# jasonleebrown/machisplin

Hardware: AMD Instinct MI355X
Metric: grid Mcells/s (ensemble+TPS predict) + TPS-solve GFLOP/s (higher is better)
Workload: dtype f64; 1 GPU; cfg3: 5000 stations, 3 covariates, 10000x10000 grid, 6-model ensemble + TPS residual correction; stations=5000, covariates=3 x float32 planes resident in HBM, rf_trees=500, tps_mode=global (one fit on all stations, GCV lambda, V73:748-753), parallelism=rowband1 + bcast(coef) + 1 all-gather

## Files before the change

machisplin_amd/csrc/ensemble.hip:

```cpp
#include <algorithm>
#include <atomic>
#include <chrono>
#include <cmath>
#include <cstdio>
#include <cstdlib>
#include <cstring>
#include <functional>
#include <mutex>
#include <type_traits>
#include <vector>
#include "common.h"
#include "devmath.h"

#include "ensemble_int.h"

namespace mhs {

__global__ __launch_bounds__(256) void lm_kernel(const double *__restrict__ coef, int p, StackDev s,
                                                 PredGeom g, double weight, int accumulate,
                                                 double *__restrict__ out) {
    const int64_t i = (int64_t)blockIdx.x * 256 + threadIdx.x;
    if (i >= (int64_t)g.nr * g.nc) return;
    const int row = (int)(i / g.nc), col = (int)(i - (int64_t)row * g.nc);
    double acc = coef[0];
// ... 64 lines not shown
    double w_lm, w_nn, w_ea;
};
template <int P>
__global__ __launch_bounds__(256) void small_members_kernel(SmallArgs a, StackDev s, PredGeom g, int accumulate,
                                                            double *__restrict__ out) {
    const int64_t i = (int64_t)blockIdx.x * 256 + threadIdx.x;
    if (i >= (int64_t)g.nr * g.nc) return;
    const int row = (int)(i / g.nc), col = (int)(i - (int64_t)row * g.nc);
    double x[P];
    bool na = false;
#pragma unroll
    for (int j = 0; j < P; ++j) { x[j] = predictor(s, g, j, row, col); na |= isnan(x[j]); }
    const int64_t o = (int64_t)row * g.ld_out + col;
    double v = accumulate ? out[o] : 0.0;
    bool first = !accumulate;
    auto add = [&](double pred, double w) { const double t = pred * w; v = first ? t : v + t; first = false; };
    if (a.lm_coef) {
        double acc = a.lm_coef[0];
#pragma unroll
        for (int j = 0; j < P; ++j) acc = acc + a.lm_coef[j + 1] * x[j];
        add(acc, a.w_lm);
    }
    if (a.nn_w) {
        double acc = a.nn_w[(P + 1) * a.nn_H];
        for (int h = 0; h < a.nn_H; ++h) {
            const double *wh = a.nn_w + h * (P + 1);
            double z = wh[0];
#pragma unroll
            for (int j = 0; j < P; ++j) z = z + wh[1 + j] * x[j];
            acc = acc + a.nn_w[(P + 1) * a.nn_H + 1 + h] * nnet_sigmoid(z);
        }
        acc = acc * a.nn_scale + a.nn_shift;
        add(na ? NAN : acc, a.w_nn);
    }
    if (a.ea_coef) {
        double acc = 0.0;
        for (int k = 0; k < a.ea_nterms; ++k) {
            double term = 1.0;
            for (int f = a.ea_tstart[k]; f < a.ea_tstart[k + 1]; ++f) {
                const double xv = predictor(s, g, a.ea_fvar[f], row, col);
                const int d = a.ea_fdir[f];
                const double fac = d == 2 ? xv : (d == 1 ? fmax(0.0, xv - a.ea_cut[f]) : fmax(0.0, a.ea_cut[f] - xv));
                term = term * fac;
            }
            acc = acc + a.ea_coef[k] * term;
        }
        add(na ? NAN : acc, a.w_ea);
    }
    out[o] = v;
}

constexpr int EXP_TAB_BITS = 12;
constexpr int EXP_TAB_N = 1 << EXP_TAB_BITS;
constexpr double EXP_SCALE = 4096.0 / 0.6931471805599453094;
constexpr double EXP_RANGE = 700.0;
__device__ __forceinline__ double table_exp_neg_acc(double u, const double *tab, double acc) {
    const double MAGIC = 0x1.8p52 + 1023.0 * EXP_TAB_N, NK = -EXP_RANGE * EXP_SCALE;
    const double t = fma(u, NK, MAGIC);
    const double kd = t - MAGIC;
    unsigned k8 = (unsigned)__double2loint(t) << 8;
    asm("" : "+v"(k8));
    const double r = fma(u, NK, -kd);
    const double mj = *(const double *)((const char *)tab + __builtin_amdgcn_ubfe(k8, 5, EXP_TAB_BITS + 3));
    const double sj = __hiloint2double((int)((k8 & 0xfff00000u) | (unsigned)__double2hiint(mj)), __double2loint(mj));
    const double C1 = 1.0 / EXP_SCALE, C2 = 0.5 / (EXP_SCALE * EXP_SCALE);
    double q = fma(r, C2, C1);
    q = fma(q, r, 1.0);
    return fma(sj, q, acc);
}

template <int P, int R>
__global__ __launch_bounds__(256) void svr_kernel(const double *__restrict__ svp, int nsv, int stride,
                                                  int npos, const double *__restrict__ xcs,
                                                  const double *__restrict__ gtab, double sigma, double b,
                                                  double amax,
                                                  double y_center, double y_scale, StackDev s, PredGeom g,
                                                  double weight, int accumulate, double *__restrict__ out) {
    __shared__ double etab[EXP_TAB_N];
    for (int i = threadIdx.x; i < EXP_TAB_N; i += 256) {
        const double e = gtab[i];
        etab[i] = __hiloint2double(__double2hiint(e) & 0x000fffff, __double2loint(e));
    }
    __syncthreads();
    const int64_t total = (int64_t)g.nr * g.nc;
    const int64_t half = (total + R - 1) / R;
    const int64_t i0 = (int64_t)blockIdx.x * 256 + threadIdx.x;
    if (i0 >= half) return;
    double x[R][P], q[R], acc[R];
    bool na[R];
    int row[R], col[R];
#pragma unroll
    for (int c = 0; c < R; ++c) {
        int64_t i = i0 + c * half;
        if (i >= total) i = total - 1;
        row[c] = (int)(i / g.nc); col[c] = (int)(i - (int64_t)row[c] * g.nc);
        na[c] = false; q[c] = 0.0; acc[c] = 0.0;
#pragma unroll
        for (int j = 0; j < P; ++j) {
            const double xv = predictor(s, g, j, row[c], col[c]);
            na[c] |= isnan(xv);
            x[c][j] = (xv - xcs[j]) / xcs[P + j];
            q[c] = fma(x[c][j], x[c][j], q[c]);
        }
        q[c] = (sigma / EXP_RANGE) * q[c];
    }
    double accn[R];
#pragma unroll
    for (int c = 0; c < R; ++c) accn[c] = 0.0;
    auto sum_range = [&](int v0, int v1, double (&a)[R]) {
        for (int v = v0; v < v1; ++v) {
            const double *sp = svp + (int64_t)v * stride;
#pragma unroll
            for (int c = 0; c < R; ++c) {
                double arg = q[c] + fma(sp[P - 1], x[c][P - 1], sp[P]);
#pragma unroll
                for (int j = 0; j < P - 1; ++j) arg = fma(sp[j], x[c][j], arg);
                arg = fmin(fmax(arg, 0.0), 1.0);
                a[c] = table_exp_neg_acc(arg, etab, a[c]);
            }
        }
    };
    sum_range(0, npos, acc);
    sum_range(npos, nsv, accn);
#pragma unroll
    for (int c = 0; c < R; ++c) {
        const int64_t i = i0 + c * half;
        if (i < total) {
            const double pred = ((acc[c] - accn[c]) * amax - b) * y_scale + y_center;
            emit(out, (int64_t)row[c] * g.ld_out + col[c], na[c] ? NAN : pred, weight, accumulate);
        }
    }
}

template <int P, int R>
__global__ __launch_bounds__(256) void svr_rt_kernel(const double *__restrict__ svp, int nsv, int stride,
                                                     int npos, const double *__restrict__ xcs,
                                                     const double *__restrict__ gtab, double sigma, double b,
                                                     double amax, double y_center, double y_scale, StackDev s, PredGeom g,
                                                     int tiles_per_row, double weight, int accumulate, double *__restrict__ out) {
    constexpr int CH = 128;
    __shared__ double etab[EXP_TAB_N];
    __shared__ double aw[4][CH];
    for (int i = threadIdx.x; i < EXP_TAB_N; i += 256) {
        const double e = gtab[i];
        etab[i] = __hiloint2double(__double2hiint(e) & 0x000fffff, __double2loint(e));
    }
    __syncthreads();
    const int wave = threadIdx.x >> 6, lane = threadIdx.x & 63;
    const int64_t ntiles = (int64_t)g.nr * tiles_per_row;
    const int64_t tile = (int64_t)blockIdx.x * 4 + wave;
    if (tile >= ntiles) return;
    const int row = (int)(tile / tiles_per_row), tcol = (int)(tile - (int64_t)row * tiles_per_row) * (64 * R);
    double x[R][P], q[R], acc[R], accn[R];
    bool na[R], ok[R];
    int col[R];
#pragma unroll
    for (int c = 0; c < R; ++c) {
        const int cc = tcol + c * 64 + lane;
        ok[c] = cc < g.nc;
        col[c] = min(cc, g.nc - 1);
        na[c] = false; q[c] = 0.0; acc[c] = 0.0; accn[c] = 0.0;
#pragma unroll
        for (int j = 0; j < P; ++j) {
            const double xv = predictor(s, g, j, row, col[c]);
            na[c] |= isnan(xv);
            x[c][j] = (xv - xcs[j]) / xcs[P + j];
            q[c] = fma(x[c][j], x[c][j], q[c]);
        }
        q[c] = (sigma / EXP_RANGE) * q[c];
    }
    const double xlat = x[0][P - 1];
    double qhi = -1.0, qlo = 2e300;
#pragma unroll
    for (int c = 0; c < R; ++c) { qhi = fmax(qhi, q[c]); qlo = fmin(qlo, q[c]); }
#pragma unroll
    for (int o = 32; o > 0; o >>= 1) { qhi = fmax(qhi, __shfl_xor(qhi, o)); qlo = fmin(qlo, __shfl_xor(qlo, o)); }
    const bool fold = __builtin_amdgcn_readfirstlane((int)(qhi - qlo <= 0.5)) != 0;
    const double S = fold ? qhi : 0.0;
    auto sum_range = [&](int v0, int v1, double (&a)[R], auto folded) {
        constexpr bool FOLD = decltype(folded)::value;
        auto pair = [&](const double *sp, const double ap) {
#pragma unroll
            for (int c = 0; c < R; ++c) {
                double arg = FOLD ? ap : q[c] + ap;
#pragma unroll
                for (int j = 0; j < P - 1; ++j) arg = fma(sp[j], x[c][j], arg);
                arg = fmin(fmax(arg, 0.0), 1.0);
                a[c] = table_exp_neg_acc(arg, etab, a[c]);
            }
        };
        for (int vb = v0; vb < v1; vb += CH) {
            const int n = min(CH, v1 - vb);
            __builtin_amdgcn_wave_barrier();
            for (int e = lane; e < n; e += 64) {
                const double *sp = svp + (int64_t)(vb + e) * stride;
                aw[wave][e] = fma(sp[P - 1], xlat, sp[P]) + S;
            }
            __builtin_amdgcn_wave_barrier();
            const double *sp = svp + (int64_t)vb * stride;
            const double *ar = aw[wave];
            int e = 0;
            for (; e + 4 <= n; e += 4) {
#pragma unroll
                for (int k = 0; k < 4; ++k) pair(sp + (int64_t)k * stride, ar[e + k]);
                sp += (int64_t)4 * stride;
            }
            for (; e < n; ++e) { pair(sp, ar[e]); sp += stride; }
        }
    };
    if (fold) {
        sum_range(0, npos, acc, std::true_type());
        sum_range(npos, nsv, accn, std::true_type());
    } else {
        sum_range(0, npos, acc, std::false_type());
        sum_range(npos, nsv, accn, std::false_type());
    }
#pragma unroll
    for (int c = 0; c < R; ++c)
        if (ok[c]) {
            const double back = fold ? exp(EXP_RANGE * (S - q[c])) : 1.0;
            const double pred = ((acc[c] - accn[c]) * back * amax - b) * y_scale + y_center;
            emit(out, (int64_t)row * g.ld_out + col[c], na[c] ? NAN : pred, weight, accumulate);
        }
}

template <bool GBM, bool LDS_NODES, int R, bool NA_ONLY, bool SPLIT = false>
__global__ __launch_bounds__(256) void tree_kernel(const Node *__restrict__ gnodes,
                                                   const int *__restrict__ tree_off,
                                                   const TreeChunk *__restrict__ chunks, int n_chunks,
                                                   int n_trees, double init_f, int p, StackDev s,
                                                   PredGeom g, double weight, int accumulate,
                                                   double *__restrict__ out, const unsigned *__restrict__ na_gate = nullptr) {
    extern __shared__ __attribute__((aligned(16))) char smem[];
    if (NA_ONLY && na_gate && na_gate[1] == 0u) return;
    double *xs = (double *)smem;
    Node *lnodes = (Node *)(smem + (size_t)p * R * 256 * sizeof(double));
    const int64_t total = (int64_t)g.nr * g.nc;
    const int64_t half = (total + R - 1) / R;
    const int64_t i0 = (int64_t)blockIdx.x * 256 + threadIdx.x;
    int row[R], col[R];
    bool na[R];
    double acc[R];
#pragma unroll
    for (int c = 0; c < R; ++c) {
        int64_t i = i0 + c * half;
        if (i >= total) i = total - 1;
        if (i < 0) i = 0;
        row[c] = (int)(i / g.nc); col[c] = (int)(i - (int64_t)row[c] * g.nc);
        na[c] = false; acc[c] = 0.0;
        for (int j = 0; j < p; ++j) {
            const double xv = predictor(s, g, j, row[c], col[c]);
            na[c] |= isnan(xv);
            xs[(j * R + c) * 256 + threadIdx.x] = xv;
        }
    }
    if (NA_ONLY) {
        bool any = false;
#pragma unroll
        for (int c = 0; c < R; ++c) any |= na[c] && i0 < half && (i0 + c * half) < total;
        if (!__syncthreads_or(any)) return;
    }
    int ch_begin = 0, ch_end = n_chunks;
    if (SPLIT) {
        const int per = (n_chunks + (int)gridDim.y - 1) / (int)gridDim.y;
        ch_begin = min((int)blockIdx.y * per, n_chunks);
        ch_end = min(ch_begin + per, n_chunks);
    }
    for (int ch = ch_begin; ch < ch_end; ++ch) {
        const TreeChunk tc = chunks[ch];
        if (LDS_NODES) {
            __syncthreads();
            const int4 *src = (const int4 *)(gnodes + tc.node_begin);
            int4 *dst = (int4 *)lnodes;
            for (int e = threadIdx.x; e < tc.node_count; e += 256) dst[e] = src[e];
            __syncthreads();
        }
        for (int t = tc.first_tree; t < tc.first_tree + tc.n_trees; ++t) {
            const int tbase = LDS_NODES ? tree_off[t] - tc.node_begin : tree_off[t];
#pragma unroll
            for (int c = 0; c < R; ++c) {
                if (NA_ONLY && !na[c]) continue;
                Node nd;
                if constexpr (LDS_NODES) nd = lnodes[tbase]; else nd = gnodes[tbase];
                while (nd.var >= 0) {
                    const double xv = xs[(nd.var * R + c) * 256 + threadIdx.x];
                    unsigned nxt;
                    if (GBM) nxt = isnan(xv) ? nd.missing : (xv < nd.val ? nd.left : nd.right);
                    else nxt = (xv <= nd.val) ? nd.left : nd.right;
                    if constexpr (LDS_NODES) nd = lnodes[tbase + nxt]; else nd = gnodes[tbase + nxt];
                }
                acc[c] = acc[c] + nd.val;
            }
        }
    }
    if (SPLIT) {
#pragma unroll
        for (int c = 0; c < R; ++c) {
            const int64_t i = i0 + c * half;
            if (i0 < half && i < total) out[(int64_t)blockIdx.y * total + i] = (!GBM && na[c]) ? NAN : acc[c];
        }
        return;
    }
#pragma unroll
    for (int c = 0; c < R; ++c) {
        const int64_t i = i0 + c * half;
        if (i0 < half && i < total && (!NA_ONLY || na[c])) {
            double pred;
            if (GBM) pred = init_f + acc[c];
            else pred = na[c] ? NAN : acc[c] / (double)n_trees;
            emit(out, (int64_t)row[c] * g.ld_out + col[c], pred, weight, accumulate);
        }
    }
}


__global__ __launch_bounds__(256) void na_collect_kernel(StackDev s, PredGeom g, unsigned cap, unsigned *__restrict__ list) {
    const int64_t total = (int64_t)g.nr * g.nc;
    const int64_t i = (int64_t)blockIdx.x * 256 + threadIdx.x;
    if (i >= total) return;
    const int row = (int)(i / g.nc), col = (int)(i - (int64_t)row * g.nc);
    bool na = false;
    for (int j = 0; j < s.C; ++j) na |= isnan(predictor(s, g, j, row, col));
    if (na) {
        const unsigned slot = atomicAdd(&list[0], 1u);
        if (slot < cap) list[2 + slot] = (unsigned)i;
        else list[1] = 1u;
    }
}
template <bool LDS_NODES>
__global__ __launch_bounds__(256) void gbm_na_list_kernel(const Node *__restrict__ gnodes, const int *__restrict__ tree_off,
                                                          const TreeChunk *__restrict__ chunks, int n_chunks, double init_f, int p,
                                                          StackDev s, PredGeom g, double weight, int accumulate,
                                                          double *__restrict__ out, const unsigned *__restrict__ list, unsigned cap) {
    extern __shared__ __attribute__((aligned(16))) char smem[];
    if (list[1]) return;
    double *xs = (double *)smem;
    Node *lnodes = (Node *)(smem + (size_t)p * 256 * sizeof(double));
    const unsigned count = min(list[0], cap);
    for (unsigned base = blockIdx.x * 256u; base < count; base += gridDim.x * 256u) {
        const bool live = base + threadIdx.x < count;
        const int64_t i = list[2 + (live ? base + threadIdx.x : base)];
        const int row = (int)(i / g.nc), col = (int)(i - (int64_t)row * g.nc);
        for (int j = 0; j < p; ++j) xs[j * 256 + threadIdx.x] = predictor(s, g, j, row, col);
        double acc = 0.0;
        for (int ch = 0; ch < n_chunks; ++ch) {
            const TreeChunk tc = chunks[ch];
            if (LDS_NODES) {
                __syncthreads();
                const int4 *src = (const int4 *)(gnodes + tc.node_begin);
                int4 *dst = (int4 *)lnodes;
                for (int e = threadIdx.x; e < tc.node_count; e += 256) dst[e] = src[e];
                __syncthreads();
            }
            for (int t = tc.first_tree; t < tc.first_tree + tc.n_trees; ++t) {
                const int tbase = LDS_NODES ? tree_off[t] - tc.node_begin : tree_off[t];
                Node nd;
                if constexpr (LDS_NODES) nd = lnodes[tbase]; else nd = gnodes[tbase];
                while (nd.var >= 0) {
                    const double xv = xs[nd.var * 256 + threadIdx.x];
                    const unsigned nxt = isnan(xv) ? nd.missing : (xv < nd.val ? nd.left : nd.right);
                    if constexpr (LDS_NODES) nd = lnodes[tbase + nxt]; else nd = gnodes[tbase + nxt];
                }
                acc = acc + nd.val;
            }
        }
        if (live) emit(out, (int64_t)row * g.ld_out + col, init_f + acc, weight, accumulate);
        __syncthreads();
    }
}


template <bool HI>
__device__ __forceinline__ void pred_bits(float2v &b01, float2v &b23, const float2v k01, const float2v k23,
                                          const unsigned long long cpair) {
    if (!HI)
        asm("v_pk_add_f32 %0, %2, %4 op_sel_hi:[1,0] clamp\n\t"
// ... 452 lines not shown
        const unsigned abase = (unsigned)buf * (unsigned)((CH << S) * sizeof(double)) - 0x58000000u;
        for (unsigned long long m2 = __builtin_amdgcn_ballot_w64(multi); m2; m2 &= m2 - 1ull) {
            const int t = (int)__builtin_ctzll(m2);
            const int n = __builtin_amdgcn_readlane((int)nstr, t);
            const float a0 = __uint_as_float(0x4B000000u + ((unsigned)t << S) + (unsigned)__builtin_amdgcn_readlane((int)known, t));
            float2v s01 = {a0, a0}, s23 = {a0, a0};
#pragma unroll
            for (int l = 0; l < S; ++l) {
                if (l < n) {
                    const unsigned long long cc = (unsigned)__builtin_amdgcn_readlane((int)cl[l], t);
                    const unsigned vw = (unsigned)__builtin_amdgcn_readlane((int)vl[l], t);
                    const int vo = (int)(vw & 0xFFu);
                    const unsigned long long wb = (127u + (vw >> 8)) << 23;
                    float2v b01, b23;
                    asm volatile("s_set_gpr_idx_on %[vo], 0x1\n\t"
                                 "v_pk_add_f32 %[b01], v[64:65], %[cc] op_sel_hi:[1,0] clamp\n\t"
                                 "v_pk_add_f32 %[b23], v[66:67], %[cc] op_sel_hi:[1,0] clamp\n\t"
                                 "s_set_gpr_idx_off\n\t"
                                 "v_pk_fma_f32 %[s01], %[b01], %[wb], %[s01] op_sel_hi:[1,0,1]\n\t"
                                 "v_pk_fma_f32 %[s23], %[b23], %[wb], %[s23] op_sel_hi:[1,0,1]"
                                 : [s01] "+v"(s01), [s23] "+v"(s23), [b01] "=&v"(b01), [b23] "=&v"(b23)
                                 : "{v[64:95]}"(keys), [vo] "s"(vo), [cc] "s"(cc), [wb] "s"(wb));
                }
            }
            acc[0] = acc[0] + gbc_lds_f64(__float_as_uint(s01.x) * 8u + abase);
            acc[1] = acc[1] + gbc_lds_f64(__float_as_uint(s01.y) * 8u + abase);
            acc[2] = acc[2] + gbc_lds_f64(__float_as_uint(s23.x) * 8u + abase);
            acc[3] = acc[3] + gbc_lds_f64(__float_as_uint(s23.y) * 8u + abase);
        }
        if (more) {
            double *ld = slut + (buf ^ 1) * (CH << S);
            ld[tid] = pre0; ld[tid + 1024] = pre1;
            if (tid < CH * S) scls[(buf ^ 1) * CLS_STRIDE + tid] = prec;
        }
        __syncthreads();
    }
    if (PROBE) {
        int *tot = (int *)srange;
        __syncthreads();
        if (tid == 0) tot[0] = 0;
        __syncthreads();
#pragma unroll
        for (int o = 32; o > 0; o >>= 1) pcost += __shfl_xor(pcost, o);
        if (lane == 0) atomicAdd(tot, pcost);
        __syncthreads();
        if (tid == 0) { probe[2 * blockIdx.x] = tot[0]; probe[2 * blockIdx.x + 1] = GBC_WAVES * n_trees_padded; }
        return;
    }
#pragma unroll
    for (int o = 32; o > 0; o >>= 1) usum = usum + __shfl_xor(usum, o);
#pragma unroll
    for (int c = 0; c < R; ++c)
        if (ok[c] && !na[c]) emit(out, (int64_t)row[c] * g.ld_out + col[c], init_f + (acc[c] + usum), weight, accumulate);
}
static size_t gbc_lds_bytes() {
    return 2 * ((size_t)LUT_CHUNK << 5) * sizeof(double) + 2 * 384 * sizeof(unsigned) + GBC_WAVES * 8 * sizeof(int2);
}

__global__ __launch_bounds__(256) void gbm_staged_points_kernel(const Node *__restrict__ nodes, const int *__restrict__ tree_off,
                                                                int n_trees, double init_f, const double *__restrict__ X,
                                                                int64_t n, int step, double *__restrict__ out) {
    const int64_t i = (int64_t)blockIdx.x * 256 + threadIdx.x;
    if (i >= n) return;
    double acc = 0.0;
    for (int t = 0; t < n_trees; ++t) {
        const int tb = tree_off[t];
        Node nd = nodes[tb];
        while (nd.var >= 0) {
            const double xv = X[(int64_t)nd.var * n + i];
            const unsigned nxt = isnan(xv) ? nd.missing : (xv < nd.val ? nd.left : nd.right);
            nd = nodes[tb + nxt];
        }
        acc = acc + nd.val;
        if ((t + 1) % step == 0) out[(int64_t)((t + 1) / step - 1) * n + i] = init_f + acc;
    }
}

struct ResidualArgs { double w[8]; };
__global__ __launch_bounds__(256) void residual_points_kernel(const double *__restrict__ pred, const double *__restrict__ resp,
                                                              int64_t n, int n_models, ResidualArgs a, double wt_total,
                                                              double *__restrict__ out) {
    const int64_t i = (int64_t)blockIdx.x * 256 + threadIdx.x;
    if (i >= n) return;
    const double y = resp[i];
    double res = (y - pred[i]) * a.w[0];
    for (int k = 1; k < n_models; ++k) res = res + (y - pred[(int64_t)k * n + i]) * a.w[k];
    out[i] = res / wt_total;
}

__global__ __launch_bounds__(256) void scale_add_kernel(const double *__restrict__ a, double divisor,
                                                        const double *__restrict__ b,
                                                        double *__restrict__ out, int64_t n) {
    const int64_t i = (int64_t)blockIdx.x * 256 + threadIdx.x;
    if (i >= n) return;
    double v = a[i] / divisor;
    if (b) v = v + b[i];
    out[i] = v;
}

__global__ __launch_bounds__(256) void scale_window_kernel(double *__restrict__ out, int nr, int nc,
                                                           int64_t ld, double divisor) {
    const int64_t i = (int64_t)blockIdx.x * 256 + threadIdx.x;
    if (i >= (int64_t)nr * nc) return;
    const int row = (int)(i / nc), col = (int)(i - (int64_t)row * nc);
    out[(int64_t)row * ld + col] = out[(int64_t)row * ld + col] / divisor;
}


int finish_trees(mhs_model *m, const std::vector<Node> &nodes, const std::vector<int> &off) {
    const int nt = m->n_trees;
    const size_t xs_bytes = (size_t)m->p * TREE_R * 256 * sizeof(double);
    int biggest = 0;
    for (int t = 0; t < nt; ++t) biggest = std::max(biggest, off[t + 1] - off[t]);
    int cap = (m->kind == K_GBM) ? std::max(GBM_CHUNK_NODES, biggest) : biggest;
    m->lds_ok = xs_bytes + (size_t)cap * sizeof(Node) <= LDS_LIMIT;
    std::vector<TreeChunk> chunks;
    if (m->lds_ok) {
        int t = 0;
        while (t < nt) {
            TreeChunk c{t, 0, off[t], 0};
            while (t < nt && off[t + 1] - c.node_begin <= cap) { ++t; }
            c.n_trees = t - c.first_tree;
            c.node_count = off[t] - c.node_begin;
            chunks.push_back(c);
        }
        m->max_chunk_nodes = cap;
    } else {
        chunks.push_back(TreeChunk{0, nt, 0, off[nt]});
        m->max_chunk_nodes = 0;
    }
    m->n_chunks = (int)chunks.size();
    m->n_nodes = (int64_t)nodes.size();
    if (int rc = to_device(nodes.data(), nodes.size(), &m->nodes)) return rc;
    if (int rc = to_device(off.data(), off.size(), &m->tree_off)) return rc;
    return to_device(chunks.data(), chunks.size(), &m->chunks);
}

int check_common(int p, mhs_model **out) {
    if (int rc = require_ready()) return rc;
    MHS_REQUIRE(out != nullptr, "out is NULL");
    MHS_REQUIRE(p >= 2 && p <= 64, "p (covariates + LONG + LAT) out of range");
    return MHS_OK;
}

template <int P>
static void launch_nnet(const mhs_model *m, const StackDev &s, const PredGeom &g, double w, int acc,
                        double *out, hipStream_t st, unsigned blocks) {
    hipLaunchKernelGGL((nnet_kernel<P>), dim3(blocks), dim3(256), 0, st, m->dpar, m->n0, m->s0, m->s1, s, g, w, acc, out);
}
template <int P>
static void launch_svr(const mhs_model *m, const StackDev &s, const PredGeom &g, double w, int acc,
                       double *out, hipStream_t st, int64_t total) {
    constexpr int R = 3;
    const int tpr = (g.nc + 64 * R - 1) / (64 * R);
    if (!s.all_from_planes && P == s.C + 2 && P >= 3 && !getenv("MHS_SVR_NO_ROWTILE") && (double)g.nc >= 0.93 * (double)tpr * (64 * R)) {
        const int64_t ntiles = (int64_t)g.nr * tpr;
        hipLaunchKernelGGL((svr_rt_kernel<P, R>), dim3((unsigned)((ntiles + 3) / 4)), dim3(256), 0, st,
                           m->dpar, m->n0, m->n1, m->n2, m->dpar + (size_t)m->n0 * m->n1, ctx().exp_tab, m->s1, m->s0, m->s4,
                           m->s2, m->s3, s, g, tpr, w, acc, out);
        return;
    }
    const int64_t half = (total + R - 1) / R;
    hipLaunchKernelGGL((svr_kernel<P, R>), dim3((unsigned)((half + 255) / 256)), dim3(256), 0, st,
                       m->dpar, m->n0, m->n1, m->n2, m->dpar + (size_t)m->n0 * m->n1, ctx().exp_tab, m->s1, m->s0, m->s4,
                       m->s2, m->s3,
                       s, g, w, acc, out);
}

#define MHS_DISPATCH_P(P_, CALL)                                                     \
    switch (P_) {                                                                    \
        case 2: CALL(2); break; case 3: CALL(3); break; case 4: CALL(4); break;      \
        case 5: CALL(5); break; case 6: CALL(6); break; case 7: CALL(7); break;      \
        case 8: CALL(8); break; case 9: CALL(9); break; case 10: CALL(10); break;    \
        case 11: CALL(11); break; case 12: CALL(12); break;                          \
        default: set_error("predict: p = %d exceeds the %d predictors this build supports for nnet/ksvm", P_, PMAX); \
                 return MHS_ERR_INVALID;                                             \
    }

template <bool GBM>
__global__ __launch_bounds__(256) void tree_finalize_kernel(const double *__restrict__ part, int shares, int64_t total,
                                                            double init_f, int n_trees, PredGeom g, double weight,
                                                            int accumulate, double *__restrict__ out) {
    const int64_t i = (int64_t)blockIdx.x * 256 + threadIdx.x;
    if (i >= total) return;
    double acc = 0.0;
    for (int y = 0; y < shares; ++y) acc = acc + part[(int64_t)y * total + i];
    const int row = (int)(i / g.nc), col = (int)(i - (int64_t)row * g.nc);
    emit(out, (int64_t)row * g.ld_out + col, GBM ? init_f + acc : acc / (double)n_trees, weight, accumulate);
}

constexpr int64_t TREE_SPLIT_MAX_CELLS = 16384;
constexpr int TREE_SPLIT_SHARES = 64;

template <bool GBM, bool NA_ONLY>
static int launch_trees(const mhs_model *m, const StackDev &s, const PredGeom &g, double w, int acc,
                        double *out, hipStream_t st, int64_t total) {
    const int64_t half = (total + TREE_R - 1) / TREE_R;
    const unsigned blocks = (unsigned)((half + 255) / 256);
    const size_t xs_bytes = (size_t)m->p * TREE_R * 256 * sizeof(double);
    if (!NA_ONLY && m->lds_ok && total <= TREE_SPLIT_MAX_CELLS && m->n_chunks >= 4) {
        const int shares = std::min(m->n_chunks, TREE_SPLIT_SHARES);
        mhs_model *mm = const_cast<mhs_model *>(m);
        if (!mm->split_scratch) MHS_HIP(hipMalloc((void **)&mm->split_scratch, sizeof(double) * TREE_SPLIT_MAX_CELLS * TREE_SPLIT_SHARES));
        const size_t bytes = xs_bytes + (size_t)m->max_chunk_nodes * sizeof(Node);
        auto kern = tree_kernel<GBM, true, TREE_R, false, true>;
        MHS_HIP(hipFuncSetAttribute((const void *)kern, hipFuncAttributeMaxDynamicSharedMemorySize, (int)bytes));
        hipLaunchKernelGGL(kern, dim3(blocks, (unsigned)shares), dim3(256), bytes, st, m->nodes, m->tree_off, m->chunks,
                           m->n_chunks, m->n_trees, m->init_f, m->p, s, g, w, acc, mm->split_scratch, (const unsigned *)nullptr);
        hipLaunchKernelGGL(tree_finalize_kernel<GBM>, dim3((unsigned)((total + 255) / 256)), dim3(256), 0, st,
                           mm->split_scratch, shares, total, m->init_f, m->n_trees, g, w, acc, out);
        return MHS_OK;
    }
    if (m->lds_ok) {
        const size_t bytes = xs_bytes + (size_t)m->max_chunk_nodes * sizeof(Node);
        auto kern = tree_kernel<GBM, true, TREE_R, NA_ONLY>;
        MHS_HIP(hipFuncSetAttribute((const void *)kern, hipFuncAttributeMaxDynamicSharedMemorySize, (int)bytes));
        hipLaunchKernelGGL(kern, dim3(blocks), dim3(256), bytes, st, m->nodes, m->tree_off, m->chunks,
                           m->n_chunks, m->n_trees, m->init_f, m->p, s, g, w, acc, out, (const unsigned *)nullptr);
    } else {
        auto kern = tree_kernel<GBM, false, TREE_R, NA_ONLY>;
        MHS_HIP(hipFuncSetAttribute((const void *)kern, hipFuncAttributeMaxDynamicSharedMemorySize, (int)xs_bytes));
        hipLaunchKernelGGL(kern, dim3(blocks), dim3(256), xs_bytes, st, m->nodes, m->tree_off, m->chunks,
                           m->n_chunks, m->n_trees, m->init_f, m->p, s, g, w, acc, out, (const unsigned *)nullptr);
    }
    return MHS_OK;
}

template <typename KT>
static int build_lut_meta_t(mhs_model *m, const mhs_grid &grid, int C) {
    const int S = m->lut_S;
    std::vector<KT> tkey((size_t)m->n_trees * S, (KT)0);
    std::vector<std::vector<KT>> sorted((size_t)m->p);
    for (int t = 0; t < m->n_trees; ++t) {
        for (int q = 0; q < S; ++q) {
            const int v = m->lut_var[(size_t)t * S + q];
            if (v < 0) continue;
            const KT tk = split_tkey<KT, false>(v, C, m->lut_thr[(size_t)t * S + q], grid);
            tkey[(size_t)t * S + q] = tk;
            sorted[(size_t)v].push_back(tk);
        }
    }
    std::vector<int> off;
    std::vector<KT> flat;
    sort_unique(sorted, off, flat);
    for (int v = 0; v < m->p; ++v)
        if (sorted[(size_t)v].size() >= ((size_t)1 << 24)) { set_error("gbm: too many distinct split values"); return MHS_ERR_INVALID; }
    if (int rc = publish_axis_ranks(m, sorted, C, grid)) return rc;
    std::vector<int> meta((size_t)m->n_trees_padded * LUT_META_DW, 0);
    const float never = -33554432.f;
    for (int t = 0; t < m->n_trees_padded; ++t) {
        int *mt = &meta[(size_t)t * LUT_META_DW];
        for (int q = 0; q < 6; ++q) { memcpy(&mt[q], &never, 4); mt[6 + q] = 0; }
        if (t >= m->n_trees) continue;
        for (int q = 0; q < S; ++q) {
            const int v = m->lut_var[(size_t)t * S + q];
            if (v < 0) continue;
            const std::vector<KT> &sv = sorted[(size_t)v];
            const KT tk = tkey[(size_t)t * S + q];
            const float c = (float)((std::lower_bound(sv.begin(), sv.end(), tk) - sv.begin()) + 1);
            memcpy(&mt[q], &c, 4);
            mt[6 + q] = v * 256 * LUT_R * (int)sizeof(float);
        }
    }
    if (m->p <= LUT_REG_P && S == 5 && !m->lut_host.empty()) {
        const int lat = C + 1 < m->p ? C + 1 : -2;
        std::vector<int> rmeta(((size_t)m->n_trees_padded + 1) * LUT_RT_DW, 0);
        std::vector<double> rlut(m->lut_host.size(), 0.0);
        for (int t = 0; t <= m->n_trees_padded; ++t) {
            int *mt = &rmeta[(size_t)t * LUT_RT_DW];
            for (int q = 0; q < 5; ++q) { memcpy(&mt[q], &never, 4); mt[6 + q] = 0; mt[11 + q] = 0; }
            mt[5] = S - LUT_RT_MAXK;
            if (t >= m->n_trees) continue;
            int perm[6], K = 0, n = 0;
            bool first[6] = {false, false, false, false, false, false};
            for (int q = 0; q < S && K < LUT_RT_MAXK; ++q) {
                const int v = m->lut_var[(size_t)t * S + q];
                if (v < 0 || v == lat) { perm[n++] = q; first[q] = true; ++K; }
            }
            for (int q = 0; q < S; ++q) if (!first[q]) perm[n++] = q;
            for (int i = 0; i < S; ++i) {
                const int q = perm[i], v = m->lut_var[(size_t)t * S + q];
                if (v < 0) continue;
                const std::vector<KT> &sv = sorted[(size_t)v];
                const int c = (int)(std::lower_bound(sv.begin(), sv.end(), tkey[(size_t)t * S + q]) - sv.begin()) + 1;
                if (i < K) mt[11 + i] = c;
                else { const float cf = (float)c; memcpy(&mt[i - K], &cf, 4); mt[6 + i - K] = v * LUT_R; }
            }
            mt[5] = S - K;
            for (int b = 0; b < (1 << S); ++b) {
                int bo = 0;
                for (int i = 0; i < S; ++i) bo |= ((b >> (S - 1 - i)) & 1) << (S - 1 - perm[i]);
                rlut[((size_t)t << S) + b] = m->lut_host[((size_t)t << S) + bo];
            }
        }
        if (int rc = publish(m, rlut, &m->lut_rt)) return rc;
        if (int rc = publish(m, rmeta, &m->lut_rt_meta)) return rc;
        std::vector<unsigned> cw((size_t)m->n_trees_padded * 5, 0u);
        for (int t = 0; t < m->n_trees; ++t)
            for (int q = 0; q < S; ++q) {
                const int v = m->lut_var[(size_t)t * S + q];
                if (v < 0) continue;
                const std::vector<KT> &sv = sorted[(size_t)v];
                const unsigned c = (unsigned)(std::lower_bound(sv.begin(), sv.end(), tkey[(size_t)t * S + q]) - sv.begin()) + 1u;
                cw[(size_t)t * 5 + q] = (c << 3) | (unsigned)v;
            }
        if (int rc = publish(m, cw, &m->lut_cls)) return rc;
    }
    if (int rc = publish(m, flat, (KT **)&m->lut_sorted)) return rc;
    if (int rc = publish(m, off, &m->lut_sorted_off)) return rc;
    return publish(m, meta, &m->lut_meta);
}

// ... 879 lines not shown
```

Measured before the change: 427.6 Mcells/s.

## Split SVR row-tile kernel into full tiles plus a packed remainder kernel

The row-tiled SVR kernel now handles only full 192-column tiles, so the per-lane bounds checks and clamping are gone. A new remainder kernel packs the leftover columns of up to 8 rows into each wave, with per-row shared lat coefficients. This avoids wasting lanes on partial tiles at the end of each row (10000 columns leave a remainder of 16 per row). The cost is a second kernel launch and a less efficient remainder path that has no fold optimisation.

```diff
diff --git a/machisplin_amd/csrc/ensemble.hip b/machisplin_amd/csrc/ensemble.hip
--- a/machisplin_amd/csrc/ensemble.hip
+++ b/machisplin_amd/csrc/ensemble.hip
@@ -240,13 +240,11 @@
     if (tile >= ntiles) return;
     const int row = (int)(tile / tiles_per_row), tcol = (int)(tile - (int64_t)row * tiles_per_row) * (64 * R);
     double x[R][P], q[R], acc[R], accn[R];
-    bool na[R], ok[R];
+    bool na[R];
     int col[R];
 #pragma unroll
     for (int c = 0; c < R; ++c) {
-        const int cc = tcol + c * 64 + lane;
-        ok[c] = cc < g.nc;
-        col[c] = min(cc, g.nc - 1);
+        col[c] = tcol + c * 64 + lane;
         na[c] = false; q[c] = 0.0; acc[c] = 0.0; accn[c] = 0.0;
 #pragma unroll
         for (int j = 0; j < P; ++j) {
@@ -304,12 +302,86 @@
         sum_range(npos, nsv, accn, std::false_type());
     }
 #pragma unroll
-    for (int c = 0; c < R; ++c)
-        if (ok[c]) {
-            const double back = fold ? exp(EXP_RANGE * (S - q[c])) : 1.0;
-            const double pred = ((acc[c] - accn[c]) * back * amax - b) * y_scale + y_center;
-            emit(out, (int64_t)row * g.ld_out + col[c], na[c] ? NAN : pred, weight, accumulate);
-        }
+    for (int c = 0; c < R; ++c) {
+        const double back = fold ? exp(EXP_RANGE * (S - q[c])) : 1.0;
+        const double pred = ((acc[c] - accn[c]) * back * amax - b) * y_scale + y_center;
+        emit(out, (int64_t)row * g.ld_out + col[c], na[c] ? NAN : pred, weight, accumulate);
+    }
+}
+
+constexpr int REM_ROWS = 8;
+static int svr_rem_cells_per_wave(int rem) { return rem >= REM_ROWS ? 64 : REM_ROWS * rem; }
+template <int P>
+__global__ __launch_bounds__(256) void svr_rem_kernel(const double *__restrict__ svp, int nsv, int stride,
+                                                      int npos, const double *__restrict__ xcs,
+                                                      const double *__restrict__ gtab, double sigma, double b,
+                                                      double amax, double y_center, double y_scale, StackDev s, PredGeom g,
+                                                      int c_first, int rem, int per_wave, double weight, int accumulate,
+                                                      double *__restrict__ out) {
+    constexpr int CH = 64;
+    __shared__ double etab[EXP_TAB_N];
+    __shared__ double aw[4][REM_ROWS][CH];
+    for (int i = threadIdx.x; i < EXP_TAB_N; i += 256) {
+        const double e = gtab[i];
+        etab[i] = __hiloint2double(__double2hiint(e) & 0x000fffff, __double2loint(e));
+    }
+    __syncthreads();
+    const int wave = __builtin_amdgcn_readfirstlane(threadIdx.x >> 6), lane = threadIdx.x & 63;
+    const int64_t ncell = (int64_t)g.nr * rem;
+    const int64_t f0 = ((int64_t)blockIdx.x * 4 + wave) * per_wave;
+    if (f0 >= ncell) return;
+    const int64_t f1 = min(f0 + per_wave, ncell) - 1;
+    const bool ok = f0 + lane <= f1;
+    const int64_t f = min(f0 + lane, f1);
+    const int row0 = (int)(f0 / rem), nrows = (int)(f1 / rem) - row0 + 1;
+    const int row = (int)(f / rem), col = c_first + (int)(f - (int64_t)row * rem);
+    double x[P], q = 0.0, acc = 0.0, accn = 0.0;
+    bool na = false;
+#pragma unroll
+    for (int j = 0; j < P; ++j) {
+        const double xv = predictor(s, g, j, row, col);
+        na |= isnan(xv);
+        x[j] = (xv - xcs[j]) / xcs[P + j];
+        q = fma(x[j], x[j], q);
+    }
+    q = (sigma / EXP_RANGE) * q;
+    const double *ar = aw[wave][row - row0];
+    auto sum_range = [&](int v0, int v1, double &a) {
+        auto pair = [&](const double *sp, const double ap) {
+            double arg = q + ap;
+#pragma unroll
+            for (int j = 0; j < P - 1; ++j) arg = fma(sp[j], x[j], arg);
+            arg = fmin(fmax(arg, 0.0), 1.0);
+            a = table_exp_neg_acc(arg, etab, a);
+        };
+        for (int vb = v0; vb < v1; vb += CH) {
+            const int n = min(CH, v1 - vb);
+            __builtin_amdgcn_wave_barrier();
+            if (lane < n) {
+                const double *sp = svp + (int64_t)(vb + lane) * stride;
+                const double bl = sp[P - 1], al = sp[P];
+                for (int r = 0; r < nrows; ++r) {
+                    const double xlat = (predictor(s, g, P - 1, row0 + r, 0) - xcs[P - 1]) / xcs[2 * P - 1];
+                    aw[wave][r][lane] = fma(bl, xlat, al);
+                }
+            }
+            __builtin_amdgcn_wave_barrier();
+            const double *sp = svp + (int64_t)vb * stride;
+            int e = 0;
+            for (; e + 4 <= n; e += 4) {
+#pragma unroll
+                for (int k = 0; k < 4; ++k) pair(sp + (int64_t)k * stride, ar[e + k]);
+                sp += (int64_t)4 * stride;
+            }
+            for (; e < n; ++e) { pair(sp, ar[e]); sp += stride; }
+        }
+    };
+    sum_range(0, npos, acc);
+    sum_range(npos, nsv, accn);
+    if (ok) {
+        const double pred = ((acc - accn) * amax - b) * y_scale + y_center;
+        emit(out, (int64_t)row * g.ld_out + col, na ? NAN : pred, weight, accumulate);
+    }
 }
 
 template <bool GBM, bool LDS_NODES, int R, bool NA_ONLY, bool SPLIT = false>
@@ -1068,12 +1140,22 @@
 static void launch_svr(const mhs_model *m, const StackDev &s, const PredGeom &g, double w, int acc,
                        double *out, hipStream_t st, int64_t total) {
     constexpr int R = 3;
-    const int tpr = (g.nc + 64 * R - 1) / (64 * R);
-    if (!s.all_from_planes && P == s.C + 2 && P >= 3 && !getenv("MHS_SVR_NO_ROWTILE") && (double)g.nc >= 0.93 * (double)tpr * (64 * R)) {
+    const int tpr_ceil = (g.nc + 64 * R - 1) / (64 * R);
+    if (!s.all_from_planes && P == s.C + 2 && P >= 3 && !getenv("MHS_SVR_NO_ROWTILE") && (double)g.nc >= 0.93 * (double)tpr_ceil * (64 * R)) {
+        const int tpr = g.nc / (64 * R), rem = g.nc - tpr * (64 * R);
         const int64_t ntiles = (int64_t)g.nr * tpr;
-        hipLaunchKernelGGL((svr_rt_kernel<P, R>), dim3((unsigned)((ntiles + 3) / 4)), dim3(256), 0, st,
-                           m->dpar, m->n0, m->n1, m->n2, m->dpar + (size_t)m->n0 * m->n1, ctx().exp_tab, m->s1, m->s0, m->s4,
-                           m->s2, m->s3, s, g, tpr, w, acc, out);
+        if (ntiles > 0) {
+            hipLaunchKernelGGL((svr_rt_kernel<P, R>), dim3((unsigned)((ntiles + 3) / 4)), dim3(256), 0, st,
+                               m->dpar, m->n0, m->n1, m->n2, m->dpar + (size_t)m->n0 * m->n1, ctx().exp_tab, m->s1, m->s0, m->s4,
+                               m->s2, m->s3, s, g, tpr, w, acc, out);
+        }
+        if (rem > 0) {
+            const int per_wave = svr_rem_cells_per_wave(rem);
+            const int64_t nwaves = ((int64_t)g.nr * rem + per_wave - 1) / per_wave;
+            hipLaunchKernelGGL((svr_rem_kernel<P>), dim3((unsigned)((nwaves + 3) / 4)), dim3(256), 0, st,
+                               m->dpar, m->n0, m->n1, m->n2, m->dpar + (size_t)m->n0 * m->n1, ctx().exp_tab, m->s1, m->s0, m->s4,
+                               m->s2, m->s3, s, g, tpr * (64 * R), rem, per_wave, w, acc, out);
+        }
         return;
     }
     const int64_t half = (total + R - 1) / R;
```

Measured after the change: 430.5 Mcells/s (median of 6 runs). No clear change (+0.7%).
